# plevankiem/model-predictive-control-for-bipedal-locomotion

Measured on AMD Instinct MI355X. Metric: QP solves/sec (horizon=150, batched) at 1/2/4/8 MI355X; CoM RMSE vs ref, higher is better.
Workload: dtype f64; 1 GPU; config2: default.json walks + rigid offsets, unconstrained, horizon=150, n=420; walks_per_gpu=4096, global_batch=4096, horizon=150, samples_per_walk=420, parallelism=dp1, strict=False

## Files before the change

### model-predictive-control-for-bipedal-locomotion_amd/csrc/rollout.hip

```cpp
#include <algorithm>
#include <climits>
#include <cstdint>
#include <cstdio>
#include <cstdlib>
#include <vector>

#include "zmpc_internal.h"

namespace {

struct Mat3 {
  double m[9];
};

__device__ __forceinline__ Mat3 matmul3(const Mat3& a, const Mat3& b) {
  Mat3 c;
#pragma unroll
  for (int i = 0; i < 3; ++i)
#pragma unroll
    for (int j = 0; j < 3; ++j)
      c.m[3 * i + j] = fma(a.m[3 * i + 0], b.m[0 + j],
                           fma(a.m[3 * i + 1], b.m[3 + j], a.m[3 * i + 2] * b.m[6 + j]));
  return c;
}
// ... 234 lines not shown
#pragma unroll
      for (int j = 0; j < 3; ++j) Ab.m[3 * i + j] = A[3 * i + j] - Bv[i] * kx[j];
  }
  const int C = REGF ? CW : (nsteps + 63) / 64;
  const int mbeg = lane * C;
  const int64_t kick_step = kick_step_of(a, b);

  double s0[3] = {0.0, 0.0, 0.0}, s1[3] = {0.0, 0.0, 0.0};
  auto scan_step = [&](int m, double fx, double fy) {
    double t[3];
    matvec3(Ab, s0, t);
    s0[0] = fma(Bv[0], fx, t[0]);
    s0[1] = fma(Bv[1], fx, t[1]);
    s0[2] = fma(Bv[2], fx, t[2]);
    matvec3(Ab, s1, t);
    s1[0] = fma(Bv[0], fy, t[0]);
    s1[1] = fma(Bv[1], fy, t[1]);
    s1[2] = fma(Bv[2], fy, t[2]);
    if (m == kick_step) s1[1] -= kk;
  };
  if constexpr (REGF) {
#pragma unroll
    for (int q = 0; q < CW; ++q)
      if (mbeg + q < nsteps) scan_step(mbeg + q, a0[q], a1[q]);
  } else {
    for (int m = mbeg; m < min(mbeg + C, nsteps); ++m) scan_step(m, f0[m], f1[m]);
  }
  Mat3 P;
  const bool pre = REGF && a.scanP != nullptr;
  if (pre) {
#pragma unroll
    for (int q = 0; q < 9; ++q) P.m[q] = a.scanP[(C - 1) * kScanStride + q];
  } else {
    P = Ab;
    for (int q = 1; q < C; ++q) P = matmul3(P, Ab);
  }
  if (lane == 0) {
    double t[3];
    matvec3(P, xi0, t);
    for (int i = 0; i < 3; ++i) s0[i] += t[i];
    matvec3(P, xi1, t);
    for (int i = 0; i < 3; ++i) s1[i] += t[i];
  }
  Mat3 Pd = P;
  int r2 = 0;
  for (int d = 1; d < (dbgb(a, 2) ? 1 : 64); d <<= 1, ++r2) {
    double u0[3], u1[3];
#pragma unroll
    for (int i = 0; i < 3; ++i) {
      u0[i] = __shfl_up(s0[i], d, 64);
      u1[i] = __shfl_up(s1[i], d, 64);
    }
    if (lane >= d) {
      double t[3];
      matvec3(Pd, u0, t);
      for (int i = 0; i < 3; ++i) s0[i] += t[i];
      matvec3(Pd, u1, t);
      for (int i = 0; i < 3; ++i) s1[i] += t[i];
    }
    if (pre && r2 < 5) {
#pragma unroll
      for (int q = 0; q < 9; ++q) Pd.m[q] = a.scanP[(C - 1) * kScanStride + (r2 + 1) * 9 + q];
    } else {
      Pd = matmul3(Pd, Pd);
    }
  }
  double x[3], y[3];
#pragma unroll
  for (int i = 0; i < 3; ++i) {
    const double p0 = __shfl_up(s0[i], 1, 64);
    const double p1 = __shfl_up(s1[i], 1, 64);
    x[i] = (lane == 0) ? xi0[i] : p0;
    y[i] = (lane == 0) ? xi1[i] : p1;
  }

  const int rows_per_round = (2 * a.lzp) / 6;
  double* hb = a.hist + b * (int64_t)n * 6;
  const double xs0[3] = {x[0], x[1], x[2]}, ys0[3] = {y[0], y[1], y[2]};
  for (int r0 = 0; r0 < n; r0 += rows_per_round) {
    const int r1 = min(r0 + rows_per_round, n);
    if (lane == 0 && r0 == 0) {
      stage[0] = xi0[0];
      stage[1] = xi0[1];
      stage[2] = xi0[2];
      stage[3] = xi1[0];
      stage[4] = xi1[1];
      stage[5] = xi1[2];
    }
#pragma unroll
    for (int i = 0; i < 3; ++i) {
      x[i] = xs0[i];
      y[i] = ys0[i];
    }
    auto replay_step = [&](int m, double fx, double fy) {
      const double ux = fx - (kx0 * x[0] + kx1 * x[1] + kx2 * x[2]);
      const double uy = fy - (kx0 * y[0] + kx1 * y[1] + kx2 * y[2]);
      double xn[3], yn[3];
      lipm_step(lc, x, ux, xn);
      lipm_step(lc, y, uy, yn);
      if (m == kick_step) yn[1] -= kk;
      const int row = m + 1;
      if (row >= r0 && row < r1) {
        double* o = stage + (row - r0) * 6;
        o[0] = xn[0];
        o[1] = xn[1];
        o[2] = xn[2];
        o[3] = yn[0];
        o[4] = yn[1];
        o[5] = yn[2];
      }
#pragma unroll
      for (int i = 0; i < 3; ++i) {
        x[i] = xn[i];
        y[i] = yn[i];
      }
    };
    if constexpr (REGF) {
#pragma unroll
      for (int q = 0; q < CW; ++q)
        if (mbeg + q < nsteps) replay_step(mbeg + q, a0[q], a1[q]);
    } else {
      for (int m = mbeg; m < min(mbeg + C, nsteps); ++m) replay_step(m, f0[m], f1[m]);
    }
    __syncthreads();
    if (!dbgb(a, 4)) {
      const int nd2 = (r1 - r0) * 3;
      const double2* src = reinterpret_cast<const double2*>(stage);
      double2* dst = reinterpret_cast<double2*>(hb + (int64_t)r0 * 6);
      for (int e = lane; e < nd2; e += 64) dst[e] = src[e];
    }
    __syncthreads();
  }
  if (a.status != nullptr) {
    const bool finite = isfinite(x[0]) && isfinite(x[1]) && isfinite(x[2]) &&
                        isfinite(y[0]) && isfinite(y[1]) && isfinite(y[2]);
    const unsigned long long bad = __ballot(!finite);
    if (lane == 0) a.status[b] = bad ? ZMPC_ST_NONFINITE : 0;
  }
}

template <int CW>
__global__ void __launch_bounds__(64) zmpc_rollout_unc_kernel(RolloutArgs a) {
  constexpr int PF = CW + 1;
  extern __shared__ __attribute__((aligned(16))) double smem[];
  const int lane = threadIdx.x;
  const int64_t b = blockIdx.x;
  double* ks = smem;
  double* zr0 = smem + a.kcp;
  double* zr1 = zr0 + a.lzp;
  BoundRegs<PF> r;
  if (!dbgb(a, 8)) load_bounds<PF>(a, b, lane, r);
  const double* xb = a.x0 + b * 6;
  const double xi0[3] = {xb[0], xb[1], xb[2]};
  const double xi1[3] = {xb[3], xb[4], xb[5]};
  const double kk = (a.kick != nullptr) ? a.kick[b] : 0.0;
  for (int j = lane; j < a.kcp; j += 64) ks[j] = a.k[j];
  store_zref<CW, PF>(a, r, zr0, zr1, lane);
  __syncthreads();
  double a0[CW], a1[CW];
  if (!dbgb(a, 1)) {
    correlate<CW>(a, ks, zr0, zr1, lane * CW, a0, a1);
  } else {
#pragma unroll
    for (int m = 0; m < CW; ++m) a0[m] = a1[m] = 0.0;
  }
  __syncthreads();
  scan_replay_store<CW, true>(a, b, lane, a0, a1, nullptr, nullptr, zr0, xi0, xi1, kk);
}

template <int CW>
struct AxisBounds {
  static constexpr int PF2 = (CW + 2) / 2;
  double2 hi[PF2], lo[PF2];
};

template <int CW>
__device__ __forceinline__ void axis_load(const RolloutArgs& a, int64_t b, int tid,
                                          AxisBounds<CW>& r) {
  const double2* zmx = reinterpret_cast<const double2*>(a.zmax + b * a.bstride);
  const double2* zmn = reinterpret_cast<const double2*>(a.zmin + b * a.bstride);
#pragma unroll
  for (int u = 0; u < AxisBounds<CW>::PF2; ++u) {
    const int t = u * 128 + tid;
    const int tc = dbgb(a, 8) ? 0 : min(t, a.n - 1);
    r.hi[u] = zmx[tc];
    r.lo[u] = zmn[tc];
  }
}

template <int CW>
__device__ __forceinline__ void axis_correlate(const RolloutArgs& a, const double* __restrict__ ks,
                                               const double* zr, int lane, double* f) {
  using ZL = ZrLayout<CW>;
  const double* z = zr + ZL::idx(lane * CW);
  double w[CW];
#pragma unroll
  for (int m = 0; m < CW; ++m) {
    f[m] = 0.0;
    w[m] = z[ZL::idx(1 + m)];
  }
  for (int j = 0; j < (dbgb(a, 1) ? 0 : a.kc); j += CW) {
#pragma unroll
    for (int jj = 0; jj < CW; ++jj) {
      const double kj = ks[j + jj];
#pragma unroll
      for (int m = 0; m < CW; ++m) f[m] = fma(kj, w[(jj + m) % CW], f[m]);
      w[jj] = z[ZL::idx(1 + jj + CW)];
    }
    z += CW + ZL::kPad;
  }
}

template <int CW>
__device__ __forceinline__ void axis_correlate_ffa(const RolloutArgs& a,
                                                   const double* __restrict__ kt,
                                                   const double* zr, int lane, double* f) {
  static_assert(CW & 1, "the fast-FIR correlation takes odd chunk widths (no LDS padding)");
  constexpr int NP = CW / 2, NA = NP + 1, NB = NP + 1, NC = NP, U = NP + 1, W = 2 * U;
  const double* g = zr + lane * CW + 1;
  double w[W], hr[U], A[NA], Bo[NB], C[NC > 0 ? NC : 1];
#pragma unroll
  for (int j = 0; j < W; ++j) w[j] = g[j];
#pragma unroll
  for (int i = 0; i < NA; ++i) {
    A[i] = 0.0;
    Bo[i] = 0.0;
  }
#pragma unroll
  for (int i = 0; i < NC; ++i) C[i] = 0.0;
#pragma unroll
  for (int i = 0; i + 1 < NC; ++i) hr[i] = w[2 * i] + w[2 * i + 1];
  const int mloop = dbgb(a, 1) ? 0 : a.kfm;
  const double* tr = kt;
  for (int m0 = 0; m0 < mloop; m0 += U, tr += 4 * U) {
#pragma unroll
    for (int mm = 0; mm < U; ++mm) {
      const double E = tr[4 * mm], O = tr[4 * mm + 1], EO = tr[4 * mm + 2];
      const int b = 2 * mm;
      if (NC > 0) hr[(mm + NC - 1) % U] = w[(b + 2 * NC - 2) % W] + w[(b + 2 * NC - 1) % W];
#pragma unroll
      for (int i = 0; i < NA; ++i) A[i] = fma(E, w[(b + 2 * i) % W], A[i]);
#pragma unroll
      for (int i = 0; i < NB; ++i) Bo[i] = fma(O, w[(b + 2 * i + 1) % W], Bo[i]);
#pragma unroll
      for (int i = 0; i < NC; ++i) C[i] = fma(EO, hr[(mm + i) % U], C[i]);
      w[b % W] = g[2 * (m0 + mm) + W];
      w[(b + 1) % W] = g[2 * (m0 + mm) + W + 1];
    }
  }
#pragma unroll
  for (int i = 0; i < NP; ++i) {
    f[2 * i] = A[i] + Bo[i];
    f[2 * i + 1] = (C[i] - A[i]) - Bo[i + 1];
  }
  f[CW - 1] = A[NP] + Bo[NP];
}

__device__ __forceinline__ double readlane_f64(double v, int l) {
  const unsigned long long u = __builtin_bit_cast(unsigned long long, v);
  const unsigned lo = __builtin_amdgcn_readlane((unsigned)u, l);
  const unsigned hi = __builtin_amdgcn_readlane((unsigned)(u >> 32), l);
  return __builtin_bit_cast(double, ((unsigned long long)hi << 32) | lo);
}

constexpr int kSparseMax = 40;

template <int CW>
__device__ __forceinline__ bool axis_correlate_sparse(const RolloutArgs& a, const double* zr,
                                                      const double* Ts, int lane, double* f) {
  using ZL = ZrLayout<CW>;
  const double* z = zr + ZL::idx(lane * CW);
  double gv[CW + 1], d[CW];
  unsigned long long mk[CW];
  int cnt = 0;
#pragma unroll
  for (int j = 0; j <= CW; ++j) gv[j] = z[ZL::idx(j)];
#pragma unroll
  for (int q = 0; q < CW; ++q) {
    d[q] = gv[q + 1] - gv[q];
    mk[q] = __ballot(d[q] != 0.0);
    cnt += __popcll(mk[q]);
  }
  if (cnt > kSparseMax) return false;
  const int N = a.hN, s = lane * CW;
  const double S0 = Ts[ksum_s0(N)];
#pragma unroll
  for (int r = 0; r < CW; ++r) f[r] = S0 * gv[r + 1];
#pragma unroll
  for (int q = 0; q < CW; ++q) {
    unsigned long long m = mk[q];
    while (m) {
      const int L = __builtin_ctzll(m);
      m &= m - 1;
      const double dv = readlane_f64(d[q], L);
      const int e = min(max(L * CW + q - s, 0), N + CW - 1);
      const double* p = Ts + e + 9 - CW;
#pragma unroll
      for (int r = 0; r < CW; ++r) f[r] = fma(p[CW - 1 - r], dv, f[r]);
    }
  }
  return true;
}

template <int CW, bool SHF, bool PM, bool FFA>
__device__ __forceinline__ void split_walk(const RolloutArgs& a, int64_t b, double* smem,
                                           int* flag, const double* __restrict__ kg,
                                           const double* __restrict__ scanP,
                                           const double* __restrict__ kxp,
                                           double* __restrict__ hist) {
  using ZL = ZrLayout<CW>;
  const int tid = threadIdx.x, lane = tid & 63, axis = tid >> 6;
  const int n = a.n, nsteps = n - 1;
  double f[CW];
  double pf0 = 0.0, pf1 = 0.0;
  tl_stamp(a, b, 0);
  const double* xb = a.x0 + b * 6 + 3 * axis;
  const double xi[3] = {xb[0], xb[1], xb[2]};
  const double kk = (axis == 1 && a.kick != nullptr) ? a.kick[b] : 0.0;
  if constexpr (SHF) {
    const double* fp = a.fsh + axis * a.fstride + lane * CW;
#pragma unroll
    for (int q = 0; q < CW; ++q) f[q] = fp[q];
  } else {
    double* zr0 = smem;
    double* zr1 = zr0 + a.lzp;
    if constexpr (PM) __builtin_amdgcn_s_setprio(3);
    AxisBounds<CW> r;
    axis_load<CW>(a, b, tid, r);
    const double2 hl = reinterpret_cast<const double2*>(a.zmax + b * a.bstride)[n - 1];
    const double2 ll = reinterpret_cast<const double2*>(a.zmin + b * a.bstride)[n - 1];
    double* Ts = smem + 2 * a.lzp;
    if (a.ksum != nullptr)
      for (int i = tid; i < ksum_rows(a.hN); i += 128) Ts[i] = a.ksum[i];
    if (a.pf_ahead > 0 && b + a.pf_ahead < a.B) {
      const double* src = (tid < 64 ? a.zmax : a.zmin) + (b + a.pf_ahead) * a.bstride;
      const int ln = tid & 63, nd = 2 * n;
      pf0 = src[min(ln * 8, nd - 1)];
      pf1 = src[min(ln * 8 + 512, nd - 1)];
    }
    if constexpr (PM) __builtin_amdgcn_s_setprio(0);
#pragma unroll
    for (int u = 0; u < AxisBounds<CW>::PF2; ++u) {
      const int t = u * 128 + tid;
      if (t < n) {
        zr0[ZL::idx(t)] = (r.hi[u].x + r.lo[u].x) / 2;
        zr1[ZL::idx(t)] = (r.hi[u].y + r.lo[u].y) / 2;
      }
    }
    {
      const double l0 = (hl.x + ll.x) / 2, l1 = (hl.y + ll.y) / 2;
      for (int t = n + tid; t < a.lz; t += 128) {
        zr0[ZL::idx(t)] = l0;
        zr1[ZL::idx(t)] = l1;
      }
    }
    __syncthreads();
    tl_stamp(a, b, 1);
    const bool sparse = a.ksum != nullptr && !dbgb(a, 1) &&
                        axis_correlate_sparse<CW>(a, axis ? zr1 : zr0, Ts, lane, f);
    if (sparse) {
    } else if constexpr (FFA && (CW & 1))
      axis_correlate_ffa<CW>(a, kg, axis ? zr1 : zr0, lane, f);
    else
      axis_correlate<CW>(a, kg, axis ? zr1 : zr0, lane, f);
    __syncthreads();
    tl_stamp(a, b, 2);
  }
  const int64_t kick_step = (axis == 1) ? kick_step_of(a, b) : -1;
  const LipmConsts lc = a.lc;
  const double kx0 = kxp[0], kx1 = kxp[1], kx2 = kxp[2];
  const int mbeg = lane * CW;
  double sv[3] = {0.0, 0.0, 0.0};
  {
    const double* Gc = scanP + kScanGOff;
#pragma unroll
    for (int q = 0; q < CW; ++q) {
      const double* gq = Gc + (CW - 1 - q) * 6;
#pragma unroll
      for (int i = 0; i < 3; ++i) sv[i] = fma(gq[i], f[q], sv[i]);
    }
    const int64_t qk = kick_step - mbeg;
    if (qk >= 0 && qk < CW && kick_step < nsteps) {
      const double* ek = Gc + (CW - 1 - (int)qk) * 6 + 3;
#pragma unroll
      for (int i = 0; i < 3; ++i) sv[i] = fma(-kk, ek[i], sv[i]);
    }
  }
  const double* Pp = scanP + (CW - 1) * kScanStride;
  if (lane == 0) {
    double t[3];
    Mat3 P;
#pragma unroll
    for (int q = 0; q < 9; ++q) P.m[q] = Pp[q];
    matvec3(P, xi, t);
    for (int i = 0; i < 3; ++i) sv[i] += t[i];
  }
  if (!dbgb(a, 2)) scan_dpp(sv, lane, Pp, scanP + kScanPowOff + (CW - 1) * 33 * 9);
  double x[3];
#pragma unroll
  for (int i = 0; i < 3; ++i) {
    const double p = dpp_f64<0x138, 0xF>(sv[i]);
    x[i] = (lane == 0) ? xi[i] : p;
  }
  double* stage = smem;
  if (lane == 0) {
    stage[3 * axis + 0] = xi[0];
    stage[3 * axis + 1] = xi[1];
    stage[3 * axis + 2] = xi[2];
  }
#pragma unroll
  for (int q = 0; q < CW; ++q) {
    const int m = mbeg + q;
    if (m < nsteps) {
      const double u = f[q] - (kx0 * x[0] + kx1 * x[1] + kx2 * x[2]);
      double xn[3];
      lipm_step(lc, x, u, xn);
      if (m == kick_step) xn[1] -= kk;
      double* o = stage + HistLayout<CW>::row(m + 1) + 3 * axis;
      o[0] = xn[0];
      o[1] = xn[1];
      o[2] = xn[2];
#pragma unroll
      for (int i = 0; i < 3; ++i) x[i] = xn[i];
    }
  }
  if (a.status != nullptr) {
    const bool finite = isfinite(x[0]) && isfinite(x[1]) && isfinite(x[2]);
    const unsigned long long bad = __ballot(!finite);
    if (lane == 0) flag[axis] = bad ? ZMPC_ST_NONFINITE : 0;
  }
  __syncthreads();
  tl_stamp(a, b, 3);
  if (!dbgb(a, 4)) {
    if constexpr (PM) __builtin_amdgcn_s_setprio(3);
    const double2* src = reinterpret_cast<const double2*>(stage);
    double2* dst = reinterpret_cast<double2*>(hist + b * (int64_t)n * 6);
    const int ne = n * 3;
    int e = tid;
    if constexpr (HistLayout<CW>::kPad == 0) {
      for (; e + 3 * 128 < ne; e += 4 * 128) {
        const double2 v0 = src[e], v1 = src[e + 128], v2 = src[e + 256], v3 = src[e + 384];
        st_nt2(&dst[e], v0);
        st_nt2(&dst[e + 128], v1);
        st_nt2(&dst[e + 256], v2);
        st_nt2(&dst[e + 384], v3);
      }
      for (; e < ne; e += 128) st_nt2(&dst[e], src[e]);
    } else {
      auto at = [](int e2) {
        const int r = e2 / 3;
        return e2 + (r >= 1 ? (r - 1) / HistLayout<CW>::kSpan : 0) * (HistLayout<CW>::kPad / 2);
      };
      for (; e + 3 * 128 < ne; e += 4 * 128) {
        const double2 v0 = src[at(e)], v1 = src[at(e + 128)], v2 = src[at(e + 256)],
                      v3 = src[at(e + 384)];
        st_nt2(&dst[e], v0);
        st_nt2(&dst[e + 128], v1);
        st_nt2(&dst[e + 256], v2);
        st_nt2(&dst[e + 384], v3);
      }
      for (; e < ne; e += 128) st_nt2(&dst[e], src[at(e)]);
    }
    if constexpr (PM) __builtin_amdgcn_s_setprio(0);
  }
  tl_stamp(a, b, 4);
  if (a.status != nullptr && tid == 0) a.status[b] = flag[0] | flag[1];
  if (a.dbg < 0) hist[tid] = pf0 + pf1;
}

__global__ void __launch_bounds__(256) zmpc_shared_f_kernel(const double* __restrict__ zmax,
                                                            const double* __restrict__ zmin,
                                                            int n, const double* __restrict__ k,
                                                            int kc, double* fsh, int fstride) {
  const int i = blockIdx.x * 256 + threadIdx.x;
  const int axis = blockIdx.y;
  if (i >= fstride) return;
  double acc = 0.0;
  for (int j = 0; j < kc; ++j) {
    const int t = min(i + 1 + j, n - 1);
    const double z = (zmax[2 * t + axis] + zmin[2 * t + axis]) / 2;
    acc = fma(k[j], z, acc);
  }
  fsh[axis * fstride + i] = acc;
}

template <int CW>
__global__ void __launch_bounds__(128, 4)
    zmpc_rollout_unc_persd_kernel(RolloutArgs a) {
  extern __shared__ __attribute__((aligned(16))) double smem[];
  __shared__ int flag[2];
  for (int64_t b = blockIdx.x; b < a.B; b += gridDim.x) {
    split_walk<CW, false, true, false>(a, b, smem, flag, a.k, a.scanP, a.kx, a.hist);
    __syncthreads();
  }
}

template <int CW, bool SHF>
__global__ void __launch_bounds__(128, 4) zmpc_rollout_unc_splitd_kernel(RolloutArgs a) {
  extern __shared__ __attribute__((aligned(16))) double smem[];
  __shared__ int flag[2];
  split_walk<CW, SHF, false, true>(a, blockIdx.x, smem, flag, (CW & 1) ? a.kffa : a.k, a.scanP,
                                   a.kx, a.hist);
}

__device__ __forceinline__ double2 cmul(double2 a, double2 b) {
  return make_double2(fma(a.x, b.x, -a.y * b.y), fma(a.x, b.y, a.y * b.x));
}

__device__ __forceinline__ void dft8(double2 (&v)[8]) {
  constexpr double h = 0.70710678118654752440;
  double2 a[4], c[4];
#pragma unroll
  for (int r = 0; r < 4; ++r) {
    a[r] = make_double2(v[r].x + v[r + 4].x, v[r].y + v[r + 4].y);
    c[r] = make_double2(v[r].x - v[r + 4].x, v[r].y - v[r + 4].y);
  }
  c[1] = make_double2((c[1].x + c[1].y) * h, (c[1].y - c[1].x) * h);
  c[2] = make_double2(c[2].y, -c[2].x);
  c[3] = make_double2((c[3].y - c[3].x) * h, -(c[3].x + c[3].y) * h);
  auto dft4 = [](const double2 (&q)[4], double2& y0, double2& y1, double2& y2, double2& y3) {
    const double2 t0 = make_double2(q[0].x + q[2].x, q[0].y + q[2].y);
    const double2 t1 = make_double2(q[0].x - q[2].x, q[0].y - q[2].y);
    const double2 t2 = make_double2(q[1].x + q[3].x, q[1].y + q[3].y);
    const double2 t3 = make_double2(q[1].y - q[3].y, q[3].x - q[1].x);
    y0 = make_double2(t0.x + t2.x, t0.y + t2.y);
    y2 = make_double2(t0.x - t2.x, t0.y - t2.y);
    y1 = make_double2(t1.x + t3.x, t1.y + t3.y);
    y3 = make_double2(t1.x - t3.x, t1.y - t3.y);
  };
  dft4(a, v[0], v[2], v[4], v[6]);
  dft4(c, v[1], v[3], v[5], v[7]);
}

template <int P>
__device__ __forceinline__ void fft8(double2 (&v)[8], double2* buf,
                                     const double2* __restrict__ tw, int tid) {
  constexpr int NF = P / 8;
  constexpr int LOGP = __builtin_ctz(P);
  constexpr int A8 = LOGP / 3;
  constexpr int RL = LOGP % 3;
  constexpr int R = 1 << RL;
  const bool act = tid < NF;
#pragma unroll
  for (int st = 0; st < A8; ++st) {
    const int Ns = 1 << (3 * st);
    const int k = tid & (Ns - 1);
    if (act) {
      if (st > 0) {
        const double2 w1 = tw[k * (kFftPT / (8 * Ns))];
        const double2 w2 = cmul(w1, w1), w3 = cmul(w2, w1), w4 = cmul(w2, w2);
        v[1] = cmul(v[1], w1);
        v[2] = cmul(v[2], w2);
        v[3] = cmul(v[3], w3);
        v[4] = cmul(v[4], w4);
        v[5] = cmul(v[5], cmul(w4, w1));
        v[6] = cmul(v[6], cmul(w4, w2));
        v[7] = cmul(v[7], cmul(w4, w3));
      }
      dft8(v);
    }
    const bool last = (st == A8 - 1) && RL == 0;
    if (!last) {
      if (act) {
        const int base = ((tid - k) << 3) + k;
#pragma unroll
        for (int r = 0; r < 8; ++r) buf[base + r * Ns] = v[r];
      }
      __syncthreads();
      if (act) {
        if (st + 1 < A8) {
#pragma unroll
          for (int r = 0; r < 8; ++r) v[r] = buf[tid + r * NF];
        } else {
#pragma unroll
          for (int m = 0; m < 8 / R; ++m)
#pragma unroll
            for (int r = 0; r < R; ++r) v[m * R + r] = buf[tid + NF * m + r * (P / R)];
        }
      }
      __syncthreads();
    }
  }
  if constexpr (RL > 0) {
    double2 y[8];
    if (act) {
#pragma unroll
      for (int m = 0; m < 8 / R; ++m) {
        const int j = tid + NF * m;
        const double2 w1 = tw[j * (kFftPT / P)];
        double2 q[4];
#pragma unroll
        for (int r = 0; r < R; ++r) q[r] = v[m * R + r];
        if constexpr (R == 2) {
          q[1] = cmul(q[1], w1);
          y[m] = make_double2(q[0].x + q[1].x, q[0].y + q[1].y);
          y[m + 4] = make_double2(q[0].x - q[1].x, q[0].y - q[1].y);
        } else {
          const double2 w2 = cmul(w1, w1), w3 = cmul(w2, w1);
          q[1] = cmul(q[1], w1);
          q[2] = cmul(q[2], w2);
          q[3] = cmul(q[3], w3);
          const double2 t0 = make_double2(q[0].x + q[2].x, q[0].y + q[2].y);
          const double2 t1 = make_double2(q[0].x - q[2].x, q[0].y - q[2].y);
          const double2 t2 = make_double2(q[1].x + q[3].x, q[1].y + q[3].y);
          const double2 t3 = make_double2(q[1].y - q[3].y, q[3].x - q[1].x);
          y[m] = make_double2(t0.x + t2.x, t0.y + t2.y);
          y[m + 2] = make_double2(t1.x + t3.x, t1.y + t3.y);
          y[m + 4] = make_double2(t0.x - t2.x, t0.y - t2.y);
          y[m + 6] = make_double2(t1.x - t3.x, t1.y - t3.y);
        }
      }
#pragma unroll
      for (int u = 0; u < 8; ++u) v[u] = y[u];
    }
  }
}

template <int P>
__device__ __forceinline__ void fft_correlate8(double2 (&v)[8], double2* buf,
                                               const double2* __restrict__ tw,
                                               const double2* __restrict__ G, int tid) {
  constexpr int NF = P / 8;
  fft8<P>(v, buf, tw, tid);
  if (tid < NF) {
#pragma unroll
    for (int u = 0; u < 8; ++u) {
      const double2 S = v[u], g = G[tid + NF * u];
      v[u] = make_double2(fma(S.x, g.x, S.y * g.y), fma(S.x, g.y, -S.y * g.x));
    }
  }
  __syncthreads();
  fft8<P>(v, buf, tw, tid);
  if (tid < NF) {
#pragma unroll
    for (int u = 0; u < 8; ++u) buf[tid + NF * u] = v[u];
  }
  __syncthreads();
}


template <int CW, int W>
__device__ __forceinline__ bool wide_correlate_sparse(const RolloutArgs& a, const double* zr,
                                                      const double* Ts, double* ld, int* lm,
                                                      int (*scnt)[W], int axis, int w, int lane,
                                                      double* f) {
  using ZL = ZrLayout<CW>;
  const int s = (w * 64 + lane) * CW;
  const double* z = zr + ZL::idx(s);
  double gv[CW + 1], d[CW];
  unsigned long long mk[CW];
  int cnt = 0;
#pragma unroll
  for (int j = 0; j <= CW; ++j) gv[j] = z[ZL::idx(j)];
#pragma unroll
  for (int q = 0; q < CW; ++q) {
    d[q] = gv[q + 1] - gv[q];
    mk[q] = __ballot(d[q] != 0.0);
    cnt += __popcll(mk[q]);
  }
  if (lane == 0) scnt[axis][w] = cnt;
  __syncthreads();
  int tot0 = 0, tot1 = 0, base = 0;
#pragma unroll
  for (int v = 0; v < W; ++v) {
    tot0 += scnt[0][v];
    tot1 += scnt[1][v];
    if (v < w) base += scnt[axis][v];
  }
  if (tot0 > kSparseMaxWide || tot1 > kSparseMaxWide || dbgb(a, 1)) return false;
  const unsigned long long lt = (1ull << lane) - 1ull;
  double* la = ld + axis * kSparseMaxWide;
  int* lma = lm + axis * kSparseMaxWide;
#pragma unroll
  for (int q = 0; q < CW; ++q) {
    if ((mk[q] >> lane) & 1ull) {
      const int pos = base + __popcll(mk[q] & lt);
      la[pos] = d[q];
      lma[pos] = s + q;
    }
    base += __popcll(mk[q]);
  }
  __syncthreads();
  const int N = a.hN, tot = axis ? tot1 : tot0;
  const double S0 = Ts[ksum_s0(N)];
#pragma unroll
  for (int r = 0; r < CW; ++r) f[r] = S0 * gv[r + 1];
  for (int c = 0; c < tot; ++c) {
    const int e = min(max(lma[c] - s, 0), N + CW - 1);
    const double dv = la[c];
    const double* p = Ts + e + 9 - CW;
#pragma unroll
    for (int r = 0; r < CW; ++r) f[r] = fma(p[CW - 1 - r], dv, f[r]);
  }
  return true;
}

template <int CW, int W, int E = 0>
__global__ void __launch_bounds__(128 * W, E == 4 ? 6 : 4) zmpc_rollout_unc_wide_kernel(RolloutArgs a) {
  using ZL = ZrLayout<CW>;
  constexpr int NT = 128 * W;
  extern __shared__ __attribute__((aligned(16))) double smem[];
  __shared__ int flag[2 * W];
  __shared__ double send[2][W][3];
  const int tid = threadIdx.x, lane = tid & 63, wv = tid >> 6;
  const int axis = wv / W, w = wv % W;
  const int64_t b = blockIdx.x;
  const int n = a.n, nsteps = n - 1;
  double* zr0 = smem;
  double* zr1 = zr0 + a.lzp;
  __shared__ int scnt[2][W];
  tl_stamp(a, b, 0);
  double* Ts = smem + 2 * a.lzp;
  double* ld = Ts + ((ksum_rows(a.hN) + 1) & ~1);
  int* lm = reinterpret_cast<int*>(ld + 2 * kSparseMaxWide);
  double f[CW];
  const int mbeg = (w * 64 + lane) * CW;
  double pf0 = 0.0, pf1 = 0.0;
  if (a.pf_ahead > 0 && b + a.pf_ahead < a.B) {
    const int nd = 2 * n, half = NT / 2, tl = tid % half;
    const double* src = (tid < half ? a.zmax : a.zmin) + (b + a.pf_ahead) * a.bstride;
    pf0 = src[min(tl * 8, nd - 1)];
    pf1 = src[min((tl + half) * 8, nd - 1)];
  }
  bool dense = true;
  if constexpr (E > 0) {
    if (a.ksum != nullptr) {
      const double2* zmx = reinterpret_cast<const double2*>(a.zmax + b * a.bstride);
      const double2* zmn = reinterpret_cast<const double2*>(a.zmin + b * a.bstride);
      constexpr int lzs = W * 64 * CW + 1, IT = (lzs + NT - 1) / NT, GB = CW >= 7 ? 2 : 4;
#pragma unroll
      for (int u0 = 0; u0 < IT; u0 += GB) {
        double2 hi[GB], lo[GB];
#pragma unroll
        for (int u = 0; u < GB; ++u) {
          const int tc = min(tid + (u0 + u) * NT, n - 1);
          hi[u] = zmx[tc];
          lo[u] = zmn[tc];
        }
        if (u0 == 0)
          for (int i = tid; i < ksum_rows(a.hN); i += NT) Ts[i] = a.ksum[i];
#pragma unroll
        for (int u = 0; u < GB; ++u) {
          const int t = tid + (u0 + u) * NT;
          if (u0 + u < IT && t < lzs) {
            zr0[ZL::idx(t)] = (hi[u].x + lo[u].x) / 2;
            zr1[ZL::idx(t)] = (hi[u].y + lo[u].y) / 2;
          }
        }
      }
      __syncthreads();
      tl_stamp(a, b, 1);
      dense = !wide_correlate_sparse<CW, W>(a, axis ? zr1 : zr0, Ts, ld, lm, scnt, axis, w, lane,
                                             f);
    }
  }
  if (!dense) {
  } else if constexpr (E > 0) {
    double2* buf = reinterpret_cast<double2*>(smem);
    const double2* zmx = reinterpret_cast<const double2*>(a.zmax + b * a.bstride);
    const double2* zmn = reinterpret_cast<const double2*>(a.zmin + b * a.bstride);
    constexpr int P = NT * E, NF = P / 8;
    double2 v[8];
    if (tid < NF) {
      double2 hi[8], lo[8];
#pragma unroll
      for (int u = 0; u < 8; ++u) {
        const int tc = min(tid + NF * u, n - 1);
        hi[u] = zmx[tc];
        lo[u] = zmn[tc];
      }
#pragma unroll
      for (int u = 0; u < 8; ++u)
        v[u] = make_double2((hi[u].x + lo[u].x) / 2, (hi[u].y + lo[u].y) / 2);
    }
    fft_correlate8<P>(v, buf, a.fft_tw, a.fft_g, tid);
#pragma unroll
    for (int q = 0; q < CW; ++q) {
      const double2 c = buf[min(mbeg + q, NT * E - 1)];
      f[q] = axis ? -c.y : c.x;
    }
  } else {
    const double2* zmx = reinterpret_cast<const double2*>(a.zmax + b * a.bstride);
    const double2* zmn = reinterpret_cast<const double2*>(a.zmin + b * a.bstride);
    for (int t0 = 0; t0 < a.lz; t0 += 4 * NT) {
      double2 hi[4], lo[4];
#pragma unroll
      for (int u = 0; u < 4; ++u) {
        const int tc = dbgb(a, 8) ? 0 : min(t0 + u * NT + tid, n - 1);
        hi[u] = zmx[tc];
        lo[u] = zmn[tc];
      }
#pragma unroll
      for (int u = 0; u < 4; ++u) {
        const int t = t0 + u * NT + tid;
        if (t < a.lz) {
          zr0[ZL::idx(t)] = (hi[u].x + lo[u].x) / 2;
          zr1[ZL::idx(t)] = (hi[u].y + lo[u].y) / 2;
        }
      }
    }
    if (a.ksum != nullptr)
      for (int i = tid; i < ksum_rows(a.hN); i += NT) Ts[i] = a.ksum[i];
    __syncthreads();
    if (a.ksum == nullptr ||
        !wide_correlate_sparse<CW, W>(a, axis ? zr1 : zr0, Ts, ld, lm, scnt, axis, w, lane, f))
// ... 131 lines not shown
      stage[3 * axis + 2] = xi[2];
    }
#pragma unroll
    for (int i = 0; i < 3; ++i) x[i] = xs0[i];
#pragma unroll
    for (int q = 0; q < CW; ++q) {
      const int m = mbeg + q;
      if (m < nsteps) {
        const double u = f[q] - (kx0 * x[0] + kx1 * x[1] + kx2 * x[2]);
        double xn[3];
        lipm_step(lc, x, u, xn);
        if (m == kick_step) xn[1] -= kk;
        const int row = m + 1;
        if (row >= r0 && row < r1) {
          double* o = stage + srow(row - r0) + 3 * axis;
          o[0] = xn[0];
          o[1] = xn[1];
          o[2] = xn[2];
        }
#pragma unroll
        for (int i = 0; i < 3; ++i) x[i] = xn[i];
      }
    }
    __syncthreads();
    if (!dbgb(a, 4)) {
      const int nd2 = (r1 - r0) * 3;
      const double2* src = reinterpret_cast<const double2*>(stage);
      double2* dst = reinterpret_cast<double2*>(hb + (int64_t)r0 * 6);
      for (int e = tid; e < nd2; e += NT)
        st_nt2(&dst[e], src[e + (HP / 2) * ((e / 3) / HS)]);
    }
    __syncthreads();
  }
  if (a.status != nullptr) {
    const bool finite = isfinite(x[0]) && isfinite(x[1]) && isfinite(x[2]);
    const unsigned long long bad = __ballot(!finite);
    if (lane == 0) flag[wv] = bad ? ZMPC_ST_NONFINITE : 0;
    __syncthreads();
    if (tid == 0) {
      int fl = 0;
      for (int v = 0; v < 2 * W; ++v) fl |= flag[v];
      a.status[b] = fl;
    }
  }
  tl_stamp(a, b, 4);
  if (a.dbg < 0) a.hist[tid] = pf0 + pf1;
}

template <int CW>
__device__ __forceinline__ void chunk_scan_replay(const RolloutArgs& a, int lane, const double* f0,
                                                  const double* f1, double* stage, int rows_pr,
                                                  double* xs, double* ys, double kk,
                                                  int64_t kstep, int64_t t0, int ns,
                                                  double* hb) {
  const LipmConsts lc = a.lc;
  const double kx0 = a.kx[0], kx1 = a.kx[1], kx2 = a.kx[2];
  const double Bv[3] = {lc.T3_6, lc.T2_2, lc.T};
  Mat3 Ab;
  {
    const double A[9] = {1.0, lc.T, lc.T2_2, 0.0, 1.0, lc.T, 0.0, 0.0, 1.0};
    const double kx[3] = {kx0, kx1, kx2};
#pragma unroll
    for (int i = 0; i < 3; ++i)
#pragma unroll
      for (int j = 0; j < 3; ++j) Ab.m[3 * i + j] = A[3 * i + j] - Bv[i] * kx[j];
  }
  const int C = (ns + 63) / 64;
  const int mbeg = lane * C, mend = min(mbeg + C, ns);
  double s0[3] = {0.0, 0.0, 0.0}, s1[3] = {0.0, 0.0, 0.0};
  for (int m = mbeg; m < mend; ++m) {
    double t[3];
    matvec3(Ab, s0, t);
    for (int i = 0; i < 3; ++i) s0[i] = fma(Bv[i], f0[m], t[i]);
    matvec3(Ab, s1, t);
    for (int i = 0; i < 3; ++i) s1[i] = fma(Bv[i], f1[m], t[i]);
    if (t0 + m == kstep) s1[1] -= kk;
  }
  Mat3 P = Ab;
  for (int q = 1; q < C; ++q) P = matmul3(P, Ab);
  if (lane == 0) {
    double t[3];
    matvec3(P, xs, t);
    for (int i = 0; i < 3; ++i) s0[i] += t[i];
    matvec3(P, ys, t);
    for (int i = 0; i < 3; ++i) s1[i] += t[i];
  }
  Mat3 Pd = P;
  for (int d = 1; d < 64; d <<= 1) {
    double u0[3], u1[3];
#pragma unroll
    for (int i = 0; i < 3; ++i) {
      u0[i] = __shfl_up(s0[i], d, 64);
      u1[i] = __shfl_up(s1[i], d, 64);
    }
    if (lane >= d) {
      double t[3];
      matvec3(Pd, u0, t);
      for (int i = 0; i < 3; ++i) s0[i] += t[i];
      matvec3(Pd, u1, t);
      for (int i = 0; i < 3; ++i) s1[i] += t[i];
    }
    Pd = matmul3(Pd, Pd);
  }
  double xb0[3], yb0[3];
#pragma unroll
  for (int i = 0; i < 3; ++i) {
    const double p0 = __shfl_up(s0[i], 1, 64);
    const double p1 = __shfl_up(s1[i], 1, 64);
    xb0[i] = (lane == 0) ? xs[i] : p0;
    yb0[i] = (lane == 0) ? ys[i] : p1;
  }
  double x[3], y[3];
  for (int r0 = 0; r0 < ns; r0 += rows_pr) {
    const int r1 = min(r0 + rows_pr, ns);
#pragma unroll
    for (int i = 0; i < 3; ++i) {
      x[i] = xb0[i];
      y[i] = yb0[i];
    }
    for (int m = mbeg; m < mend; ++m) {
      const double ux = f0[m] - (kx0 * x[0] + kx1 * x[1] + kx2 * x[2]);
      const double uy = f1[m] - (kx0 * y[0] + kx1 * y[1] + kx2 * y[2]);
      double xn[3], yn[3];
      lipm_step(lc, x, ux, xn);
      lipm_step(lc, y, uy, yn);
      if (t0 + m == kstep) yn[1] -= kk;
      if (m >= r0 && m < r1) {
        double* o = stage + (m - r0) * 6;
        o[0] = xn[0];
        o[1] = xn[1];
        o[2] = xn[2];
        o[3] = yn[0];
        o[4] = yn[1];
        o[5] = yn[2];
      }
#pragma unroll
      for (int i = 0; i < 3; ++i) {
        x[i] = xn[i];
        y[i] = yn[i];
      }
    }
    __syncthreads();
    const double2* src = reinterpret_cast<const double2*>(stage);
    double2* dst = reinterpret_cast<double2*>(hb + (t0 + r0 + 1) * 6);
    for (int e = lane; e < (r1 - r0) * 3; e += 64) st_nt2(&dst[e], src[e]);
    __syncthreads();
  }
  const int last = (ns - 1) / C;
#pragma unroll
  for (int i = 0; i < 3; ++i) {
    xs[i] = __shfl(x[i], last, 64);
    ys[i] = __shfl(y[i], last, 64);
  }
}

template <int CW>
__global__ void __launch_bounds__(64) zmpc_rollout_unc_chunk_kernel(RolloutArgs a, int lc) {
  using ZL = ZrLayout<CW>;
  extern __shared__ __attribute__((aligned(16))) double smem[];
  const int64_t b = blockIdx.x;
  const int lane = threadIdx.x;
  const int n = a.n;
  const int64_t nsteps = n - 1;
  double* ks = smem;
  double* zr0 = smem + a.kcp;
  double* zr1 = zr0 + a.lzp;
  double* f0 = zr1 + a.lzp;
  double* f1 = f0 + lc;
  const int rows_pr = (2 * a.lzp) / 6;
  for (int j = lane; j < a.kcp; j += 64) ks[j] = a.k[j];
  const double2* zmx = reinterpret_cast<const double2*>(a.zmax + b * a.bstride);
  const double2* zmn = reinterpret_cast<const double2*>(a.zmin + b * a.bstride);
  const double* xb = a.x0 + b * 6;
  double xs[3] = {xb[0], xb[1], xb[2]}, ys[3] = {xb[3], xb[4], xb[5]};
  const double kk = (a.kick != nullptr) ? a.kick[b] : 0.0;
  const int64_t kstep = kick_step_of(a, b);
  double* hb = a.hist + b * (int64_t)n * 6;
  if (lane < 6) hb[lane] = xb[lane];
  for (int64_t t0 = 0; t0 < nsteps; t0 += lc) {
    const int ns = (int)min((int64_t)lc, nsteps - t0);
    const int passes = (ns + 64 * CW - 1) / (64 * CW);
    const int lz = passes * 64 * CW + a.kc + 1;
    __syncthreads();
    for (int t = lane; t < lz; t += 64) {
      const int64_t row = min(t0 + t, (int64_t)n - 1);
      const double2 h = zmx[row], l = zmn[row];
      zr0[ZL::idx(t)] = (h.x + l.x) / 2;
      zr1[ZL::idx(t)] = (h.y + l.y) / 2;
    }
    __syncthreads();
    for (int pass = 0; pass < passes; ++pass) {
      const int i0 = pass * 64 * CW + lane * CW;
      double a0[CW], a1[CW];
      correlate<CW>(a, ks, zr0, zr1, i0, a0, a1);
#pragma unroll
      for (int m = 0; m < CW; ++m) {
        if (i0 + m < ns) {
          f0[i0 + m] = a0[m];
          f1[i0 + m] = a1[m];
        }
      }
    }
    __syncthreads();
    chunk_scan_replay<CW>(a, lane, f0, f1, zr0, rows_pr, xs, ys, kk, kstep, t0, ns, hb);
  }
  if (a.status != nullptr) {
    const bool finite = isfinite(xs[0]) && isfinite(xs[1]) && isfinite(xs[2]) &&
                        isfinite(ys[0]) && isfinite(ys[1]) && isfinite(ys[2]);
    if (lane == 0) a.status[b] = finite ? 0 : ZMPC_ST_NONFINITE;
  }
}

__global__ void __launch_bounds__(256) zmpc_step_unc_kernel(
    int64_t B, int N, LipmConsts lc, const double* __restrict__ k, const double* __restrict__ kxp,
    const double* __restrict__ x, const double* __restrict__ zmax_win,
    const double* __restrict__ zmin_win, double* __restrict__ x_next,
    int32_t* __restrict__ status) {
  const int64_t b = (int64_t)blockIdx.x * 4 + (threadIdx.x >> 6);
  const int lane = threadIdx.x & 63;
  if (b >= B) return;
  const double* zx = zmax_win + b * N;
  const double* zn = zmin_win + b * N;
  double acc = 0.0;
  for (int j = lane; j < N; j += 64) acc = fma(k[j], (zx[j] + zn[j]) / 2, acc);
  for (int off = 32; off > 0; off >>= 1) acc += __shfl_xor(acc, off, 64);
  if (lane == 0) {
    const double* xb = x + b * 3;
    const double xs[3] = {xb[0], xb[1], xb[2]};
    const double u = acc - (kxp[0] * xs[0] + kxp[1] * xs[1] + kxp[2] * xs[2]);
    double y[3];
    lipm_step(lc, xs, u, y);
    x_next[b * 3 + 0] = y[0];
    x_next[b * 3 + 1] = y[1];
    x_next[b * 3 + 2] = y[2];
    if (status != nullptr)
      status[b] = (isfinite(y[0]) && isfinite(y[1]) && isfinite(y[2])) ? 0 : ZMPC_ST_NONFINITE;
  }
}

int occupancy(const void* kernel, int threads, size_t lds) {
  struct Entry {
    const void* k;
    size_t lds;
    int threads, occ;
  };
  static thread_local Entry cache[32];
  static thread_local int used = 0;
  const int n = used < 32 ? used : 32;
  for (int i = 0; i < n; ++i)
    if (cache[i].k == kernel && cache[i].lds == lds && cache[i].threads == threads)
      return cache[i].occ;
  int occ = 0;
  if (hipOccupancyMaxActiveBlocksPerMultiprocessor(&occ, kernel, threads, lds) != hipSuccess)
    occ = 0;
  cache[used++ % 32] = Entry{kernel, lds, threads, occ};
  return occ;
}


template <int C, int W, int E>
void launch_wide(const UncChoice& c, hipStream_t s, RolloutArgs q, int cus) {
  const int occ = occupancy(reinterpret_cast<const void*>(zmpc_rollout_unc_wide_kernel<C, W, E>),
                            128 * W, c.lds);
  const int64_t R = (int64_t)std::max(cus, 1) * occ;
  q.pf_ahead = (R > 0 && q.n <= 512 * W && q.B <= 2 * R) ? R : 0;
  hipLaunchKernelGGL((zmpc_rollout_unc_wide_kernel<C, W, E>), dim3((unsigned)q.B), dim3(128 * W),
                     c.lds, s, q);
}

template <int C, int W>
void launch_wide_e(const UncChoice& c, hipStream_t s, const RolloutArgs& q, int cus) {
  if (c.E == 4) return launch_wide<C, W, 4>(c, s, q, cus);
  if constexpr (8 * 128 * W * 16 <= 64 * 1024) {
    if (c.E == 8) return launch_wide<C, W, 8>(c, s, q, cus);
  }
  launch_wide<C, W, 0>(c, s, q, cus);
}

template <int CW>
void launch_unc(const UncChoice& c, hipStream_t s, RolloutArgs a, int cus) {
  if (c.kind == UncKind::SplitShared) {
    hipLaunchKernelGGL((zmpc_rollout_unc_splitd_kernel<CW, true>), dim3((unsigned)a.B),
                       dim3(128), c.lds, s, a);
    return;
  }
  if (c.kind == UncKind::Generic) {
    hipLaunchKernelGGL(zmpc_rollout_unc_kernel<CW>, dim3((unsigned)a.B), dim3(64), c.lds, s, a);
    return;
  }
#ifdef ZMPC_DIAG
  static const bool pers = getenv("ZMPC_PERSISTENT") != nullptr;
  if ((CW & 1) == 0 && pers) {
    const int per_cu = occupancy(
        reinterpret_cast<const void*>(zmpc_rollout_unc_persd_kernel<CW>), 128, c.lds);
    const int64_t grid = (int64_t)std::max(cus, 1) * per_cu;
    if (per_cu > 0 && grid < a.B && a.B <= 3 * grid) {
      hipLaunchKernelGGL(zmpc_rollout_unc_persd_kernel<CW>, dim3((unsigned)grid), dim3(128),
                         c.lds, s, a);
      return;
    }
  }
#endif
  const int occ = occupancy(
      reinterpret_cast<const void*>(zmpc_rollout_unc_splitd_kernel<CW, false>), 128, c.lds);
  const int64_t R = (int64_t)std::max(cus, 1) * occ;
  a.pf_ahead = (R > 0 && a.n <= 512 && a.B <= 2 * R) ? R : 0;
  hipLaunchKernelGGL((zmpc_rollout_unc_splitd_kernel<CW, false>), dim3((unsigned)a.B),
                     dim3(128), c.lds, s, a);
}

}

#ifdef ZMPC_DIAG
static void tl_write(const unsigned long long* tl, int64_t B, hipStream_t s, hipError_t e) {
  const char* path = getenv("ZMPC_ROLLOUT_TL");
  if (tl == nullptr || path == nullptr || e != hipSuccess) return;
  std::vector<unsigned long long> h((size_t)B * 5);
  (void)hipStreamSynchronize(s);
  (void)hipMemcpy(h.data(), tl, h.size() * 8, hipMemcpyDeviceToHost);
  if (FILE* f = fopen(path, "wb")) {
    fwrite(h.data(), 8, h.size(), f);
    fclose(f);
  }
}
#endif

hipError_t zmpc_launch_rollout_unc(const zmpc_plan* p, const RolloutCall& rc, hipStream_t s,
                                   std::string* why) {
  const UncChoice c = choose_unc(p->N, rc.n, rc.bstride == 0, p->opt[ZMPC_OPT_ROLLOUT_KERNEL],
                                 p->opt[ZMPC_OPT_LONG_WALK], p->opt[ZMPC_OPT_CORRELATION]);
#ifdef ZMPC_DIAG
  static const int dbg = [] {
    const char* e = getenv("ZMPC_DEBUG_ROLLOUT");
    return e ? atoi(e) : 0;
  }();
#else
  constexpr int dbg = 0;
#endif
  RolloutArgs a{};
  a.kc = c.kc;
  a.kcp = c.kcp;
  a.lz = c.lz;
  a.lzp = c.lzp;
  a.n = (int)rc.n;
  a.B = rc.B;
  a.lc = p->lc;
  a.k = p->k;
  a.kx = p->kx;
  a.zmax = rc.zmax;
  a.zmin = rc.zmin;
  a.bstride = rc.bstride;
  a.x0 = rc.x0;
  a.kick = rc.kick;
  a.kick_step = rc.kick_step;
  a.hist = rc.hist;
  a.status = rc.status;
  a.scanP = p->scanP;
  a.dbg = dbg;
  a.kick_steps = rc.kick_steps;
  a.kffa = p->kffa;
  a.kfm = c.kfm;
  a.ksum = c.sparse ? p->ksum : nullptr;
  a.hN = p->N;
  a.fstride = c.fstride;
  if (c.E) {
    a.fft_tw = reinterpret_cast<const double2*>(p->fft_tw);
    a.fft_g = reinterpret_cast<const double2*>(p->fft_g) + (c.P - kFftPmin);
  }
#ifdef ZMPC_DIAG
  static unsigned long long* tl_buf = nullptr;
  static int64_t tl_cap = 0;
  if (getenv("ZMPC_ROLLOUT_TL") && rc.B > tl_cap) {
    if (tl_buf) (void)hipFree(tl_buf);
    tl_buf = nullptr;
    tl_cap = hipMalloc((void**)&tl_buf, (size_t)rc.B * 5 * 8) == hipSuccess ? rc.B : 0;
  }
  if (tl_buf && c.kind != UncKind::Copy && c.kind != UncKind::Chunk) {
    (void)hipMemsetAsync(tl_buf, 0, (size_t)rc.B * 5 * 8, s);
    a.tl = tl_buf;
  }
#endif
  double* fsh = nullptr;
  switch (c.kind) {
    case UncKind::Copy: {
      hipError_t e = hipMemcpyAsync(rc.hist, rc.x0, 6 * sizeof(double) * (size_t)rc.B,
                                    hipMemcpyDeviceToDevice, s);
      if (e != hipSuccess) return e;
      if (rc.status) return hipMemsetAsync(rc.status, 0, sizeof(int32_t) * rc.B, s);
      return hipSuccess;
    }
    case UncKind::Chunk:
      hipLaunchKernelGGL(zmpc_rollout_unc_chunk_kernel<8>, dim3((unsigned)a.B), dim3(64), c.lds,
                         s, a, c.lc);
      break;
    case UncKind::Wide:
      switch (c.w * 16 + c.cw) {
#define ZMPC_WCASE(W, C)                     \
  case W * 16 + C:                           \
    launch_wide_e<C, W>(c, s, a, p->cus);    \
    break;
        ZMPC_WCASE(2, 5) ZMPC_WCASE(2, 6) ZMPC_WCASE(2, 7) ZMPC_WCASE(2, 8)
        ZMPC_WCASE(4, 5) ZMPC_WCASE(4, 6) ZMPC_WCASE(4, 7) ZMPC_WCASE(4, 8)
        ZMPC_WCASE(8, 5) ZMPC_WCASE(8, 6) ZMPC_WCASE(8, 7) ZMPC_WCASE(8, 8)
#undef ZMPC_WCASE
        default:
          return hipErrorInvalidValue;
      }
      break;
    case UncKind::SplitShared: {
      const hipError_t e = hipMallocAsync((void**)&fsh, 2 * (size_t)c.fstride * sizeof(double), s);
      if (e != hipSuccess) {
        (void)hipGetLastError();
        return hipErrorOutOfMemory;
      }
      hipLaunchKernelGGL(zmpc_shared_f_kernel, dim3((unsigned)((c.fstride + 255) / 256), 2),
                         dim3(256), 0, s, rc.zmax, rc.zmin, (int)rc.n, p->k, c.kc, fsh, c.fstride);
      a.fsh = fsh;
    }
      [[fallthrough]];
    case UncKind::Split:
    case UncKind::Generic:
      switch (c.cw) {
#define ZMPC_CW(C)                      \
  case C:                               \
    launch_unc<C>(c, s, a, p->cus);     \
    break;
        ZMPC_CW(1) ZMPC_CW(2) ZMPC_CW(3) ZMPC_CW(4) ZMPC_CW(5) ZMPC_CW(6) ZMPC_CW(7) ZMPC_CW(8)
#undef ZMPC_CW
        default:
          if (fsh) (void)hipFreeAsync(fsh, s);
          return hipErrorInvalidValue;
      }
      break;
  }
  hipError_t e = hipGetLastError();
#ifdef ZMPC_DIAG
  tl_write(a.tl, rc.B, s, e);
#endif
  if (fsh) {
    const hipError_t ef = hipFreeAsync(fsh, s);
    if (e == hipSuccess) e = ef;
  }
  return e;
}

hipError_t zmpc_launch_step_unc(const zmpc_plan* p, const StepCall& c, hipStream_t s) {
  hipLaunchKernelGGL(zmpc_step_unc_kernel, dim3((unsigned)((c.B + 3) / 4)), dim3(256), 0, s, c.B,
                     p->N, p->lc, p->k, p->kx, c.x, c.zmax_win, c.zmin_win, c.x_next, c.status);
  return hipGetLastError();
}

hipError_t zmpc_rollout_unc_set_attrs() {
  hipError_t e = hipSuccess;
#define ZMPC_ATTR(C)                                                                        \
  if (e == hipSuccess)                                                                      \
    e = hipFuncSetAttribute((const void*)zmpc_rollout_unc_kernel<C>,                       \
                            hipFuncAttributeMaxDynamicSharedMemorySize, 160 * 1024);
  ZMPC_ATTR(1) ZMPC_ATTR(2) ZMPC_ATTR(3) ZMPC_ATTR(4) ZMPC_ATTR(5) ZMPC_ATTR(6) ZMPC_ATTR(7)
  ZMPC_ATTR(8)
#undef ZMPC_ATTR
  if (e == hipSuccess)
    e = hipFuncSetAttribute((const void*)zmpc_rollout_unc_chunk_kernel<8>,
                            hipFuncAttributeMaxDynamicSharedMemorySize, 160 * 1024);
#define ZMPC_WATTR(C, E)                                                                      \
  if (e == hipSuccess)                                                                        \
    e = hipFuncSetAttribute((const void*)zmpc_rollout_unc_wide_kernel<C, 8, E>,              \
                            hipFuncAttributeMaxDynamicSharedMemorySize, (int)wide_lds_cap(8));
  ZMPC_WATTR(5, 0) ZMPC_WATTR(6, 0) ZMPC_WATTR(7, 0) ZMPC_WATTR(8, 0)
  ZMPC_WATTR(5, 4) ZMPC_WATTR(6, 4) ZMPC_WATTR(7, 4) ZMPC_WATTR(8, 4)
#undef ZMPC_WATTR
  return e;
}
```

Baseline: 129.0 billion QP solves/s.

## Hoist global loads before LDS staging and defer next-walk prefetch past correlation

Rearranges the split rollout kernel so that all global loads are issued together at kernel entry: bounds, last-row targets, the first ksum rows and kick data. They are then written to LDS afterwards. The prefetch of a later walk's bounds moves to after the correlation phase behind a compile-time PFB flag, selected at launch only when prefetch-ahead is enabled. It also makes kick handling wave-uniform and branch-light, and replaces the predicated zr writes with clamped unconditional ones. The aim is to expose more memory-level parallelism and shorten the load-latency critical path. The cost is higher register pressure from holding the loads live longer.

```diff
diff --git a/model-predictive-control-for-bipedal-locomotion_amd/csrc/rollout.hip b/model-predictive-control-for-bipedal-locomotion_amd/csrc/rollout.hip
--- a/model-predictive-control-for-bipedal-locomotion_amd/csrc/rollout.hip
+++ b/model-predictive-control-for-bipedal-locomotion_amd/csrc/rollout.hip
@@ -560,7 +560,7 @@
   return true;
 }
 
-template <int CW, bool SHF, bool PM, bool FFA>
+template <int CW, bool SHF, bool PM, bool FFA, bool PFB>
 __device__ __forceinline__ void split_walk(const RolloutArgs& a, int64_t b, double* smem,
                                            int* flag, const double* __restrict__ kg,
                                            const double* __restrict__ scanP,
@@ -569,48 +569,64 @@
   using ZL = ZrLayout<CW>;
   const int tid = threadIdx.x, lane = tid & 63, axis = tid >> 6;
   const int n = a.n, nsteps = n - 1;
+  const double* Gc = scanP + kScanGOff;
   double f[CW];
   double pf0 = 0.0, pf1 = 0.0;
+  AxisBounds<CW> r;
+  double2 hl, ll;
+  double ts0 = 0.0, ts1 = 0.0;
   tl_stamp(a, b, 0);
+  if constexpr (PM && !SHF) __builtin_amdgcn_s_setprio(3);
   const double* xb = a.x0 + b * 6 + 3 * axis;
   const double xi[3] = {xb[0], xb[1], xb[2]};
-  const double kk = (axis == 1 && a.kick != nullptr) ? a.kick[b] : 0.0;
+  const double kks = (a.kick != nullptr) ? a.kick[b] : 0.0;
   if constexpr (SHF) {
     const double* fp = a.fsh + axis * a.fstride + lane * CW;
 #pragma unroll
     for (int q = 0; q < CW; ++q) f[q] = fp[q];
   } else {
+    axis_load<CW>(a, b, tid, r);
+    hl = reinterpret_cast<const double2*>(a.zmax + b * a.bstride)[n - 1];
+    ll = reinterpret_cast<const double2*>(a.zmin + b * a.bstride)[n - 1];
+    {
+      const double* tp = a.ksum != nullptr ? a.ksum : kg;
+      const int tl = a.ksum != nullptr ? ksum_rows(a.hN) - 1 : 0;
+      ts0 = tp[min(tid, tl)];
+      ts1 = tp[min(tid + 128, tl)];
+    }
+  }
+  if constexpr (PM && !SHF) __builtin_amdgcn_s_setprio(0);
+  const bool ywave = __builtin_amdgcn_readfirstlane(axis) != 0;
+  const int64_t kick_step = kick_step_of(a, b);
+  const bool kicked = ywave && kick_step >= 0 && kick_step < nsteps;
+  const int ksi = kicked ? (int)kick_step : 0;
+  const int kl = ksi / CW, qk0 = ksi - kl * CW, qk = kicked ? qk0 : -1;
+  const double* ekp = Gc + (CW - 1 - qk0) * 6 + 3;
+  const double ek[3] = {ekp[0], ekp[1], ekp[2]};
+  const double kk = (kicked && lane == kl) ? kks : 0.0;
+  if constexpr (!SHF) {
     double* zr0 = smem;
     double* zr1 = zr0 + a.lzp;
-    if constexpr (PM) __builtin_amdgcn_s_setprio(3);
-    AxisBounds<CW> r;
-    axis_load<CW>(a, b, tid, r);
-    const double2 hl = reinterpret_cast<const double2*>(a.zmax + b * a.bstride)[n - 1];
-    const double2 ll = reinterpret_cast<const double2*>(a.zmin + b * a.bstride)[n - 1];
     double* Ts = smem + 2 * a.lzp;
-    if (a.ksum != nullptr)
-      for (int i = tid; i < ksum_rows(a.hN); i += 128) Ts[i] = a.ksum[i];
-    if (a.pf_ahead > 0 && b + a.pf_ahead < a.B) {
-      const double* src = (tid < 64 ? a.zmax : a.zmin) + (b + a.pf_ahead) * a.bstride;
-      const int ln = tid & 63, nd = 2 * n;
-      pf0 = src[min(ln * 8, nd - 1)];
-      pf1 = src[min(ln * 8 + 512, nd - 1)];
-    }
-    if constexpr (PM) __builtin_amdgcn_s_setprio(0);
+    constexpr int kRows = 128 * AxisBounds<CW>::PF2;
 #pragma unroll
     for (int u = 0; u < AxisBounds<CW>::PF2; ++u) {
-      const int t = u * 128 + tid;
-      if (t < n) {
-        zr0[ZL::idx(t)] = (r.hi[u].x + r.lo[u].x) / 2;
-        zr1[ZL::idx(t)] = (r.hi[u].y + r.lo[u].y) / 2;
-      }
+      const int t = min(u * 128 + tid, a.lz - 1);
+      zr0[ZL::idx(t)] = (r.hi[u].x + r.lo[u].x) / 2;
+      zr1[ZL::idx(t)] = (r.hi[u].y + r.lo[u].y) / 2;
     }
     {
       const double l0 = (hl.x + ll.x) / 2, l1 = (hl.y + ll.y) / 2;
-      for (int t = n + tid; t < a.lz; t += 128) {
+      for (int t = kRows + tid; t < a.lz; t += 128) {
         zr0[ZL::idx(t)] = l0;
         zr1[ZL::idx(t)] = l1;
       }
+    }
+    if (a.ksum != nullptr) {
+      const int rows = ksum_rows(a.hN);
+      if (tid < rows) Ts[tid] = ts0;
+      if (tid + 128 < rows) Ts[tid + 128] = ts1;
+      for (int i = tid + 256; i < rows; i += 128) Ts[i] = a.ksum[i];
     }
     __syncthreads();
     tl_stamp(a, b, 1);
@@ -623,25 +639,29 @@
       axis_correlate<CW>(a, kg, axis ? zr1 : zr0, lane, f);
     __syncthreads();
     tl_stamp(a, b, 2);
-  }
-  const int64_t kick_step = (axis == 1) ? kick_step_of(a, b) : -1;
+    if constexpr (PFB) {
+      const double* src = (tid < 64 ? a.zmax : a.zmin) + min(b + a.pf_ahead, a.B - 1) * a.bstride;
+      const int ln = tid & 63, nd = 2 * n;
+      pf0 = src[min(ln * 8, nd - 1)];
+      pf1 = src[min(ln * 8 + 512, nd - 1)];
+    }
+  }
   const LipmConsts lc = a.lc;
   const double kx0 = kxp[0], kx1 = kxp[1], kx2 = kxp[2];
   const int mbeg = lane * CW;
   double sv[3] = {0.0, 0.0, 0.0};
   {
-    const double* Gc = scanP + kScanGOff;
 #pragma unroll
     for (int q = 0; q < CW; ++q) {
       const double* gq = Gc + (CW - 1 - q) * 6;
 #pragma unroll
       for (int i = 0; i < 3; ++i) sv[i] = fma(gq[i], f[q], sv[i]);
     }
-    const int64_t qk = kick_step - mbeg;
-    if (qk >= 0 && qk < CW && kick_step < nsteps) {
-      const double* ek = Gc + (CW - 1 - (int)qk) * 6 + 3;
-#pragma unroll
-      for (int i = 0; i < 3; ++i) sv[i] = fma(-kk, ek[i], sv[i]);
+    if (kicked) {
+      if (lane == kl) {
+#pragma unroll
+        for (int i = 0; i < 3; ++i) sv[i] = fma(-kk, ek[i], sv[i]);
+      }
     }
   }
   const double* Pp = scanP + (CW - 1) * kScanStride;
@@ -673,7 +693,7 @@
       const double u = f[q] - (kx0 * x[0] + kx1 * x[1] + kx2 * x[2]);
       double xn[3];
       lipm_step(lc, x, u, xn);
-      if (m == kick_step) xn[1] -= kk;
+      if (q == qk) xn[1] -= kk;
       double* o = stage + HistLayout<CW>::row(m + 1) + 3 * axis;
       o[0] = xn[0];
       o[1] = xn[1];
@@ -748,17 +768,17 @@
   extern __shared__ __attribute__((aligned(16))) double smem[];
   __shared__ int flag[2];
   for (int64_t b = blockIdx.x; b < a.B; b += gridDim.x) {
-    split_walk<CW, false, true, false>(a, b, smem, flag, a.k, a.scanP, a.kx, a.hist);
+    split_walk<CW, false, true, false, false>(a, b, smem, flag, a.k, a.scanP, a.kx, a.hist);
     __syncthreads();
   }
 }
 
-template <int CW, bool SHF>
+template <int CW, bool SHF, bool PFB = false>
 __global__ void __launch_bounds__(128, 4) zmpc_rollout_unc_splitd_kernel(RolloutArgs a) {
   extern __shared__ __attribute__((aligned(16))) double smem[];
   __shared__ int flag[2];
-  split_walk<CW, SHF, false, true>(a, blockIdx.x, smem, flag, (CW & 1) ? a.kffa : a.k, a.scanP,
-                                   a.kx, a.hist);
+  split_walk<CW, SHF, false, true, PFB>(a, blockIdx.x, smem, flag, (CW & 1) ? a.kffa : a.k,
+                                        a.scanP, a.kx, a.hist);
 }
 
 __device__ __forceinline__ double2 cmul(double2 a, double2 b) {
@@ -1496,11 +1516,15 @@
   }
 #endif
   const int occ = occupancy(
-      reinterpret_cast<const void*>(zmpc_rollout_unc_splitd_kernel<CW, false>), 128, c.lds);
+      reinterpret_cast<const void*>(zmpc_rollout_unc_splitd_kernel<CW, false, true>), 128, c.lds);
   const int64_t R = (int64_t)std::max(cus, 1) * occ;
   a.pf_ahead = (R > 0 && a.n <= 512 && a.B <= 2 * R) ? R : 0;
-  hipLaunchKernelGGL((zmpc_rollout_unc_splitd_kernel<CW, false>), dim3((unsigned)a.B),
-                     dim3(128), c.lds, s, a);
+  if (a.pf_ahead > 0)
+    hipLaunchKernelGGL((zmpc_rollout_unc_splitd_kernel<CW, false, true>), dim3((unsigned)a.B),
+                       dim3(128), c.lds, s, a);
+  else
+    hipLaunchKernelGGL((zmpc_rollout_unc_splitd_kernel<CW, false>), dim3((unsigned)a.B),
+                       dim3(128), c.lds, s, a);
 }
 
 }
```

New measurement: 137.7 billion QP solves/s, median of 6. 1.07x the previous value.
